# heliaxdev/ark-plonk

Measured on AMD Instinct MI355X. Metric: proofs/sec at 2^20 constraints (BLS12-381, KZG10); MSM G1-adds/s, higher is better.
Workload: dtype u32 limbs (256/384-bit Montgomery integers)

## Files before the change

### ark_plonk_amd/csrc/fieldu.cuh

```cuda
#pragma once
#include "field_common.cuh"

template <class P>
struct Fu {
    static constexpr int NL = P::NL;
    static constexpr int SAT = P::SAT_WORDS;
    static constexpr uint32_t M = (1u << 29) - 1u;
    uint32_t v[NL];

    ZK_HD static Fu zero() {
        Fu r;
#pragma unroll
        for (int i = 0; i < NL; ++i) r.v[i] = 0;
        return r;
    }
    ZK_HD static Fu one() {
        Fu r;
#pragma unroll
        for (int i = 0; i < NL; ++i) r.v[i] = P::ONE(i);
        return r;
    }
    ZK_HD bool limbs_zero() const {
        uint32_t o = 0;
#pragma unroll
        for (int i = 0; i < NL; ++i) o |= v[i];
        return o == 0;
    }

    ZK_HD static void normalize(Fu& t) {
#pragma unroll
        for (int i = 0; i < NL - 1; ++i) {
            uint32_t c = (uint32_t)((int32_t)t.v[i] >> 29);
            t.v[i] &= M;
            t.v[i + 1] += c;
        }
    }

    ZK_HD static Fu add(const Fu& a, const Fu& b) {
        Fu t;
#pragma unroll
        for (int i = 0; i < NL; ++i) t.v[i] = a.v[i] + b.v[i];
        normalize(t);
        return t;
    }
    ZK_HD static Fu dbl(const Fu& a) {
        Fu t;
#pragma unroll
        for (int i = 0; i < NL; ++i) t.v[i] = a.v[i] << 1;
        normalize(t);
        return t;
    }
    ZK_HD static Fu add3(const Fu& a, const Fu& b, const Fu& c) {
        Fu t;
#pragma unroll
        for (int i = 0; i < NL; ++i) t.v[i] = a.v[i] + b.v[i] + c.v[i];
        normalize(t);
        return t;
    }
    ZK_HD static Fu sub2(const Fu& a, const Fu& b) {
        Fu t;
#pragma unroll
        for (int i = 0; i < NL; ++i) t.v[i] = a.v[i] - b.v[i] + P::Z2(i);
        normalize(t);
        return t;
    }
    ZK_HD static Fu sub8(const Fu& a, const Fu& b) {
        Fu t;
#pragma unroll
        for (int i = 0; i < NL; ++i) t.v[i] = a.v[i] - b.v[i] + P::Z8(i);
        normalize(t);
        return t;
    }
    ZK_HD static Fu sub16(const Fu& a, const Fu& b) {
        Fu t;
#pragma unroll
        for (int i = 0; i < NL; ++i) t.v[i] = a.v[i] - b.v[i] + P::Z16(i);
        normalize(t);
        return t;
    }
    ZK_HD static Fu neg16(const Fu& a) {
        Fu t;
#pragma unroll
        for (int i = 0; i < NL; ++i) t.v[i] = P::Z16(i) - a.v[i];
        normalize(t);
        return t;
    }
    ZK_HD static Fu neg_canonical(const Fu& a) {
        Fu t;
#pragma unroll
        for (int i = 0; i < NL; ++i) t.v[i] = P::ZP(i) - a.v[i];
        normalize(t);
        return t;
    }

    ZK_HD static void sweep(Fu& t) {
#pragma unroll
        for (int i = 0; i < NL - 1; ++i) {
            const uint32_t c = t.v[i] >> 29;
            t.v[i] &= M;
            t.v[i + 1] += c;
        }
    }
    ZK_HD static Fu add_raw(const Fu& a, const Fu& b) {
        Fu t;
#pragma unroll
        for (int i = 0; i < NL; ++i) t.v[i] = a.v[i] + b.v[i];
        return t;
    }
    ZK_HD static Fu sub_raw3(const Fu& a, const Fu& b) {
        Fu t;
#pragma unroll
        for (int i = 0; i < NL; ++i) t.v[i] = a.v[i] + P::ZB3(i) - b.v[i];
        return t;
    }
    ZK_HD static Fu sub_raw8(const Fu& a, const Fu& b) {
        Fu t;
#pragma unroll
        for (int i = 0; i < NL; ++i) t.v[i] = a.v[i] + P::ZB8(i) - b.v[i];
        return t;
    }
    ZK_HD static Fu sub_raw16(const Fu& a, const Fu& b) {
        Fu t;
#pragma unroll
        for (int i = 0; i < NL; ++i) t.v[i] = a.v[i] + P::ZB16(i) - b.v[i];
        return t;
    }

    ZK_HD static Fu mul(const Fu& a, const Fu& b) {
        uint32_t m[NL];
        Fu r;
        uint64_t carry = 0;
#pragma unroll
        for (int k = 0; k < NL; ++k) {
            uint64_t a0 = 0, a1 = 0, am = 0;
#pragma unroll
            for (int i = 0; i <= k; ++i) {
                if (i & 1) a1 += (uint64_t)a.v[i] * b.v[k - i];
                else a0 += (uint64_t)a.v[i] * b.v[k - i];
            }
#pragma unroll
            for (int i = 0; i < k; ++i) am += (uint64_t)m[i] * P::MOD(k - i);
            uint64_t t = a0 + a1 + am + carry;
            m[k] = ((uint32_t)t * P::PINV) & M;
            t += (uint64_t)m[k] * P::MOD(0);
            carry = t >> 29;
        }
#pragma unroll
        for (int k = NL; k < 2 * NL - 1; ++k) {
            uint64_t a0 = 0, a1 = 0, am = 0;
#pragma unroll
            for (int i = k - NL + 1; i < NL; ++i) {
                if (i & 1) a1 += (uint64_t)a.v[i] * b.v[k - i];
                else a0 += (uint64_t)a.v[i] * b.v[k - i];
                am += (uint64_t)m[i] * P::MOD(k - i);
            }
            uint64_t t = a0 + a1 + am + carry;
            r.v[k - NL] = (uint32_t)t & M;
            carry = t >> 29;
        }
        r.v[NL - 1] = (uint32_t)carry;
        return r;
    }
    ZK_HD static uint64_t fence64(uint64_t t) {
#if defined(__HIP_DEVICE_COMPILE__)
        asm("" : "+v"(t));
#endif
        return t;
    }
    ZK_HD static Fu mul_fenced(const Fu& a, const Fu& b) {
        uint32_t m[NL];
        Fu r;
        uint64_t carry = 0;
#pragma unroll
        for (int k = 0; k < NL; ++k) {
            uint64_t t = fence64(carry + (uint64_t)a.v[0] * b.v[k]);
#pragma unroll
            for (int i = 1; i <= k; ++i) t += (uint64_t)a.v[i] * b.v[k - i];
#pragma unroll
            for (int i = 0; i < k; ++i) t += (uint64_t)m[i] * P::MOD(k - i);
            m[k] = ((uint32_t)t * P::PINV) & M;
            t += (uint64_t)m[k] * P::MOD(0);
            carry = t >> 29;
        }
#pragma unroll
        for (int k = NL; k < 2 * NL - 1; ++k) {
            uint64_t t = fence64(carry + (uint64_t)a.v[k - NL + 1] * b.v[NL - 1]);
#pragma unroll
            for (int i = k - NL + 2; i < NL; ++i) t += (uint64_t)a.v[i] * b.v[k - i];
#pragma unroll
            for (int i = k - NL + 1; i < NL; ++i) t += (uint64_t)m[i] * P::MOD(k - i);
            r.v[k - NL] = (uint32_t)t & M;
            carry = t >> 29;
        }
        r.v[NL - 1] = (uint32_t)carry;
        return r;
    }
    ZK_HD static Fu sqr(const Fu& a) {
        uint32_t m[NL], a2[NL];
        Fu r;
#pragma unroll
        for (int i = 0; i < NL; ++i) a2[i] = a.v[i] << 1;
        uint64_t carry = 0;
#pragma unroll
        for (int k = 0; k < NL; ++k) {
            uint64_t aa = 0, am = 0;
#pragma unroll
            for (int i = 0; 2 * i < k; ++i) aa += (uint64_t)a2[i] * a.v[k - i];
            if ((k & 1) == 0) aa += (uint64_t)a.v[k / 2] * a.v[k / 2];
#pragma unroll
            for (int i = 0; i < k; ++i) am += (uint64_t)m[i] * P::MOD(k - i);
            uint64_t t = aa + am + carry;
            m[k] = ((uint32_t)t * P::PINV) & M;
            t += (uint64_t)m[k] * P::MOD(0);
            carry = t >> 29;
        }
#pragma unroll
        for (int k = NL; k < 2 * NL - 1; ++k) {
            uint64_t aa = 0, am = 0;
#pragma unroll
            for (int i = k - NL + 1; 2 * i < k; ++i) aa += (uint64_t)a2[i] * a.v[k - i];
            if ((k & 1) == 0) aa += (uint64_t)a.v[k / 2] * a.v[k / 2];
#pragma unroll
            for (int i = k - NL + 1; i < NL; ++i) am += (uint64_t)m[i] * P::MOD(k - i);
            uint64_t t = aa + am + carry;
            r.v[k - NL] = (uint32_t)t & M;
            carry = t >> 29;
        }
        r.v[NL - 1] = (uint32_t)carry;
        return r;
    }

    ZK_HD bool is_zero_mod_reduced() const {
        if (v[0] != 0 && v[0] != P::MOD(0)) return false;
        uint32_t dz = 0, dp = 0;
#pragma unroll
        for (int i = 0; i < NL; ++i) {
            dz |= v[i];
            dp |= v[i] ^ P::MOD(i);
        }
        return dz == 0 || dp == 0;
    }
    ZK_HD bool is_zero_mod() const { return mul(*this, one()).is_zero_mod_reduced(); }

    ZK_HD static Fu canonical_lt2p(const Fu& a) {
        Fu d;
#pragma unroll
        for (int i = 0; i < NL; ++i) d.v[i] = a.v[i] - P::MOD(i);
        normalize(d);
        const bool neg = ((int32_t)d.v[NL - 1]) < 0;
        Fu r;
#pragma unroll
        for (int i = 0; i < NL; ++i) r.v[i] = neg ? a.v[i] : d.v[i];
        return r;
    }

    ZK_HD static Fu from_sat(const uint32_t* w) {
        Fu t = split_words(w);
        Fu c;
#pragma unroll
        for (int i = 0; i < NL; ++i) c.v[i] = P::C_IN(i);
        return mul(t, c);
    }
    ZK_HD void to_sat(uint32_t* w) const {
        Fu c;
#pragma unroll
        for (int i = 0; i < NL; ++i) c.v[i] = P::C_OUT(i);
        Fu t = canonical_lt2p(mul(*this, c));
        t.pack_words(w);
    }
    ZK_HD static Fu split_words(const uint32_t* w) {
        Fu t;
#pragma unroll
        for (int i = 0; i < NL; ++i) {
            const int bit = 29 * i;
            const int wi = bit >> 5, off = bit & 31;
            uint64_t lo = wi < SAT ? w[wi] : 0u;
            uint64_t hi = (wi + 1) < SAT ? w[wi + 1] : 0u;
            t.v[i] = (uint32_t)(((hi << 32) | lo) >> off) & M;
        }
        return t;
    }
    ZK_HD void pack_words(uint32_t* w) const { zk_pack_words<29>(*this, w); }

    ZK_HD static Fu pow_words(const Fu& a, const uint32_t* e, int n) { return zk_pow_words(a, e, n); }
    ZK_HD static Fu inverse(const Fu& a) {
        Fu pm;
#pragma unroll
        for (int i = 0; i < NL; ++i) pm.v[i] = P::MOD(i);
        uint32_t e[SAT];
        pm.pack_words(e);
        zk_words_minus_two(e);
        return zk_pow_words(a, e, SAT);
    }
};
```

### ark_plonk_amd/csrc/ntt.hip

```cpp
#include "ctx.h"
#include "domain.cuh"

#include "ntt_pass.cuh"

namespace {

template <class Fr>
struct PowBits {
    Fr p[32];
};
template <class Fr>
__global__ void gen_pow_table(void* out, uint64_t n, PowBits<Fr> pb, Fr mul, int mode, uint32_t log_m, uint32_t log_mprev, Fr to_rp) {
    uint64_t i = (uint64_t)blockIdx.x * blockDim.x + threadIdx.x;
    if (i >= n) return;
    uint64_t e = i;
    if (mode == 1) {
        uint64_t col = i & ((1ull << log_m) - 1);
        uint64_t k = i >> log_m;
        e = (col * k) & ((1ull << log_mprev) - 1);
    }
    Fr r = mul;
    for (int b = 0; b < 32; ++b) {
        if ((e >> b) & 1ull) r = Fr::mul(r, pb.p[b]);
    }
    st_fr<Fr>(out, i, Fr::mul(r, to_rp));
}

template <class FU>
__global__ void split_table(const void* packed, void* out, uint64_t n) {
    const uint64_t i = (uint64_t)blockIdx.x * blockDim.x + threadIdx.x;
    if (i >= n) return;
    const FU x = ld_u<FU>(packed, i);
    uint32_t w[4 * TW_INNER_U4];
#pragma unroll
    for (int k = 0; k < 4 * TW_INNER_U4; ++k) w[k] = k < FU::NL ? x.v[k] : 0u;
    uint4* q = reinterpret_cast<uint4*>(out) + TW_INNER_U4 * i;
#pragma unroll
    for (int k = 0; k < TW_INNER_U4; ++k) q[k] = make_uint4(w[4 * k], w[4 * k + 1], w[4 * k + 2], w[4 * k + 3]);
}

template <class Fr>
__global__ void ntt_tiny(const void* in, void* out, uint64_t in_len, uint32_t log_n, Fr w , Fr pre_g ,
                         Fr post_g , Fr scale ) {
    if (threadIdx.x != 0 || blockIdx.x != 0) return;
    const uint32_t n = 1u << log_n;
    Fr x[4], y[4];
    Fr gp = Fr::one();
    for (uint32_t i = 0; i < n; ++i) {
        x[i] = i < in_len ? Fr::mul(ld_fr<Fr>(in, i), gp) : Fr::zero();
        gp = Fr::mul(gp, pre_g);
    }
    Fr wi = Fr::one(), pg = scale;
    for (uint32_t i = 0; i < n; ++i) {
        Fr acc = Fr::zero(), wij = Fr::one();
        for (uint32_t j = 0; j < n; ++j) {
            acc = Fr::add(acc, Fr::mul(x[j], wij));
            wij = Fr::mul(wij, wi);
        }
        y[i] = Fr::mul(acc, pg);
        pg = Fr::mul(pg, post_g);
        wi = Fr::mul(wi, w);
    }
    for (uint32_t i = 0; i < n; ++i) st_fr<Fr>(out, i, y[i]);
}

template <class Fr>
__global__ void fr_convert_kernel(const void* in, void* out, uint64_t n, int to_mont) {
    uint64_t i = (uint64_t)blockIdx.x * blockDim.x + threadIdx.x;
    if (i >= n) return;
    Fr x = ld_fr<Fr>(in, i);
    st_fr<Fr>(out, i, to_mont ? Fr::to_mont(x) : Fr::from_mont(x));
}
template <class Fr>
__global__ void fr_mul_kernel(const void* a, const void* b, void* out, uint64_t n) {
    uint64_t i = (uint64_t)blockIdx.x * blockDim.x + threadIdx.x;
    if (i >= n) return;
    st_fr<Fr>(out, i, Fr::mul(ld_fr<Fr>(a, i), ld_fr<Fr>(b, i)));
}

template <class Fr>
PowBits<Fr> make_powbits(Fr base) {
    PowBits<Fr> pb;
    Fr cur = base;
    for (int b = 0; b < 32; ++b) {
        pb.p[b] = cur;
        cur = Fr::sqr(cur);
    }
    return pb;
}

template <class C>
int launch_pow_table(zk_ctx* c, void* out, uint64_t n, typename C::Fr base, typename C::Fr mul, int mode, uint32_t log_m,
                     uint32_t log_mprev) {
    typedef typename C::Fr Fr;
    if (n == 0) return ZK_OK;
    PowBits<Fr> pb = make_powbits(base);
    const Fr to_rp = to_rprime(Fr::one());
    const int T = 256;
    uint64_t blocks = (n + T - 1) / T;
    hipLaunchKernelGGL(gen_pow_table<Fr>, dim3((unsigned)blocks), dim3(T), 0, c->stream, out, n, pb, mul, mode, log_m, log_mprev, to_rp);
    ZK_HIP_TRY(hipGetLastError());
    return ZK_OK;
}

bool decompose(uint32_t log_n, int forced, int& n_pass, int s[4]) {
    s[0] = s[1] = s[2] = s[3] = 0;
    if (forced == 0 && log_n <= 9) {
        n_pass = 1;
        s[0] = (int)log_n;
        return true;
    }
    n_pass = forced ? forced : (int)((log_n + 8) / 9);
    if (n_pass > 4) return true;
    int base = (int)log_n / n_pass, extra = (int)log_n % n_pass;
    for (int i = 0; i < n_pass; ++i) s[i] = base + (i < extra ? 1 : 0);
    return forced == 0 || (s[n_pass - 1] >= 3 && s[0] <= 9);
}
int forced_passes(const zk_ctx* c, uint32_t log_n) { return log_n < 3 ? 0 : c->tune.ntt_passes; }

template <class C>
int get_inner_tw(zk_ctx* c, int s, bool inverse, void** out) {
    typedef typename C::Fr Fr;
    uint64_t key = ((uint64_t)C::ID << 40) | ((uint64_t)(inverse ? 1 : 0) << 32) | (uint64_t)s;
    auto it = c->inner_tw.find(key);
    if (it != c->inner_tw.end()) {
        *out = it->second;
        return ZK_OK;
    }
    uint64_t cnt = s >= 1 ? (1ull << (s - 1)) : 1;
    void* packed = nullptr;
    void* p = nullptr;
    ZK_HIP_TRY(hipMalloc(&packed, cnt * sizeof(Fr)));
    if (hipMalloc(&p, cnt * TW_INNER_U4 * 16) != hipSuccess) {
        (void)hipFree(packed);
        return ZK_ERR_OOM;
    }
    Fr w = domain_root<C>((uint32_t)s);
    if (inverse) w = Fr::inverse(w);
    int rc = launch_pow_table<C>(c, packed, cnt, w, Fr::one(), 0, 0, 0);
    if (!rc) {
        const int T = 256;
        hipLaunchKernelGGL(split_table<typename C::FrU>, dim3((unsigned)((cnt + T - 1) / T)), dim3(T), 0, c->stream, packed, p, cnt);
        if (hipGetLastError() != hipSuccess || hipStreamSynchronize(c->stream) != hipSuccess) rc = ZK_ERR_HIP;
    }
    (void)hipFree(packed);
    if (rc) {
        (void)hipFree(p);
        return rc;
    }
    c->inner_tw[key] = p;
    *out = p;
    return ZK_OK;
}

template <class C>
int get_plan(zk_ctx* c, uint32_t log_n, bool inverse, NttPlan** out) {
    typedef typename C::Fr Fr;
    const int forced = forced_passes(c, log_n);
    uint64_t key = ((uint64_t)C::ID << 40) | ((uint64_t)forced << 36) | ((uint64_t)(inverse ? 1 : 0) << 32) | log_n;
    auto it = c->plans.find(key);
    if (it != c->plans.end()) {
        *out = it->second;
        return ZK_OK;
    }
    int n_pass, s[4];
    if (!decompose(log_n, forced, n_pass, s)) return ZK_ERR_UNSUPPORTED;
    NttPlan* pl = new NttPlan();
    pl->curve = C::ID;
    pl->log_n = log_n;
    pl->inverse = inverse;
    pl->n_pass = n_pass;
    for (int i = 0; i < 4; ++i) pl->s[i] = s[i];
    uint32_t log_mprev = log_n;
    for (int p = 0; p < pl->n_pass; ++p) {
        if (log_n >= 3) {
            int rc = get_inner_tw<C>(c, pl->s[p], inverse, &pl->tw_inner[p]);
            if (rc) { delete pl; return rc; }
        }
        if (p + 1 < pl->n_pass) {
            uint32_t log_m = log_mprev - (uint32_t)pl->s[p];
            uint64_t cnt = 1ull << log_mprev;
            hipError_t e = hipMalloc(&pl->tw_pass[p], cnt * sizeof(Fr));
            if (e != hipSuccess) { delete pl; return ZK_ERR_OOM; }
            Fr w = domain_root<C>(log_mprev);
            if (inverse) w = Fr::inverse(w);
            int rc = launch_pow_table<C>(c, pl->tw_pass[p], cnt, w, Fr::one(), 1, log_m, log_mprev);
            if (rc) { delete pl; return rc; }
            log_mprev = log_m;
        }
    }
    c->plans[key] = pl;
    *out = pl;
    return ZK_OK;
}

template <class C>
int ensure_coset(zk_ctx* c, bool inv, uint64_t len, void** out) {
    typedef typename C::Fr Fr;
    DevBuf& buf = inv ? c->coset_inv_pow[C::ID] : c->coset_pow[C::ID];
    size_t& have = inv ? c->coset_inv_len[C::ID] : c->coset_len[C::ID];
    if (have < len) {
        ZK_HIP_TRY(hipStreamSynchronize(c->stream));
        uint64_t want = 1;
        while (want < len) want <<= 1;
        int rc = buf.ensure(want * sizeof(Fr));
        if (rc) return rc;
        Fr g = coset_gen<C>();
        if (inv) g = Fr::inverse(g);
        rc = launch_pow_table<C>(c, buf.p, want, g, Fr::one(), 0, 0, 0);
        if (rc) return rc;
        have = want;
    }
    *out = buf.p;
    return ZK_OK;
}

typedef int (*NttPassLauncher)(int final_pass, const NttPassArgs* a, hipStream_t st);
extern "C" NttPassLauncher zk_ntt_pass_launcher(int curve, int s);

template <class C>
int dispatch_pass(zk_ctx* c, int s, bool final_pass, const NttPassArgs& a) {
    if (s < 3 || s > 9) return ZK_ERR_UNSUPPORTED;
    NttPassLauncher fn = zk_ntt_pass_launcher(C::ID, s);
    if (!fn) return ZK_ERR_UNSUPPORTED;
    hipError_t e = (hipError_t)fn(final_pass ? 1 : 0, &a, c->stream);
    ZK_HIP_TRY(e);
    return ZK_OK;
}

template <class C>
int ntt_run(zk_ctx* c, int kind, uint32_t log_n, uint32_t n_polys, const void* const* d_ins, const size_t* in_lens, void* const* d_outs) {
    typedef typename C::Fr Fr;
    if (!domain_log_ok<C>(log_n)) return ZK_ERR_DOMAIN_TOO_LARGE;
    if (n_polys == 0 || n_polys > 16) return ZK_ERR_BAD_ARG;
    const uint64_t N = 1ull << log_n;
    size_t in_len = 0;
    bool all_quarter = true;
    for (uint32_t i = 0; i < n_polys; ++i) {
        if (in_lens[i] > N) return ZK_ERR_BAD_ARG;
        if (in_lens[i] > in_len) in_len = in_lens[i];
        if ((uint64_t)in_lens[i] * 4 > N) all_quarter = false;
    }
    const void* d_in = d_ins[0];
    void* d_out = d_outs[0];
    const bool inverse = (kind == ZK_NTT_IFFT || kind == ZK_NTT_COSET_IFFT);
    int rc;
    Fr n_inv = Fr::inverse(Fr::from_u64(N));
    if (log_n < 3) {
        Fr w = domain_root<C>(log_n);
        if (inverse) w = Fr::inverse(w);
        Fr g = coset_gen<C>();
        Fr pre_g = kind == ZK_NTT_COSET_FFT ? g : Fr::one();
        Fr post_g = kind == ZK_NTT_COSET_IFFT ? Fr::inverse(g) : Fr::one();
        ProfScope ps(c, "ntt_pass");
        for (uint32_t i = 0; i < n_polys; ++i)
            hipLaunchKernelGGL(ntt_tiny<Fr>, dim3(1), dim3(64), 0, c->stream, d_ins[i], d_outs[i], (uint64_t)in_lens[i], log_n, w, pre_g, post_g,
                               inverse ? n_inv : Fr::one());
        ZK_HIP_TRY(hipGetLastError());
        return ZK_OK;
    }
    {
        int np, sp[4];
        if (!decompose(log_n, forced_passes(c, log_n), np, sp)) return ZK_ERR_UNSUPPORTED;
    }
    void* pre = nullptr;
    void* post = nullptr;
    if (kind == ZK_NTT_COSET_FFT && in_len > 0) {
        rc = ensure_coset<C>(c, false, in_len, &pre);
        if (rc) return rc;
    }
    if (kind == ZK_NTT_COSET_IFFT) {
        rc = ensure_coset<C>(c, true, N, &post);
        if (rc) return rc;
    }
    NttPlan* pl = nullptr;
    rc = get_plan<C>(c, log_n, inverse, &pl);
    if (rc) return rc;
    if (pl->n_pass > 4) return ZK_ERR_UNSUPPORTED;
    void* work = nullptr;
    if (pl->n_pass > 1) {
        rc = c->ntt_work.ensure((size_t)n_polys * N * sizeof(Fr));
        if (rc) return rc;
        work = c->ntt_work.p;
    }
    uint32_t log_mprev = log_n;
    NttPassArgs a;
    ProfScope ps(c, "ntt_pass");
    for (int p = 0; p < pl->n_pass; ++p) {
        const int s = pl->s[p];
        const bool last = (p + 1 == pl->n_pass);
        memset(&a, 0, sizeof a);
        a.log_n = log_n;
        a.in = (p == 0) ? d_in : work;
        a.out = last ? d_out : work;
        a.in_len = (p == 0) ? in_lens[0] : N;
        if (n_polys > 1) {
            a.n_batch = n_polys;
            for (uint32_t i = 0; i < n_polys; ++i) {
                void* wk = (char*)work + (size_t)i * N * sizeof(Fr);
                a.ins[i] = (p == 0) ? d_ins[i] : wk;
                a.outs[i] = last ? d_outs[i] : wk;
                a.in_lens[i] = (p == 0) ? in_lens[i] : N;
            }
        }
        a.tw_inner = pl->tw_inner[p];
        a.pre_mul = (p == 0) ? pre : nullptr;
        const uint32_t LC = 9u - (uint32_t)s;
        if (!last) {
            uint32_t log_m = log_mprev - (uint32_t)s;
            uint32_t logc = LC < log_m ? LC : log_m;
            a.logc = logc;
            a.log_m = log_m;
            a.log_mprev = log_mprev;
            a.tw_pass = pl->tw_pass[p];
            a.n_tiles = (uint32_t)(N >> ((uint32_t)s + logc));
            a.quarter = (p == 0 && s >= 3 && all_quarter) ? 1u : 0u;
            log_mprev = log_m;
        } else {
            uint32_t s1 = (pl->n_pass > 1) ? (uint32_t)pl->s[0] : 0;
            uint32_t logc = LC < s1 ? LC : s1;
            a.logc = logc;
            a.s1 = s1;
            a.s2 = pl->n_pass == 4 ? (uint32_t)pl->s[1] : 0u;
            a.post_mul = post;
            const Fr sc = to_rprime(inverse ? n_inv : Fr::one());
            for (int i = 0; i < 8; ++i) a.scale[i] = sc.v[i];
            a.n_tiles = (uint32_t)(N >> ((uint32_t)s + logc));
        }
        rc = dispatch_pass<C>(c, s, last, a);
        if (rc) return rc;
        if (c->profiling) c->prof["ntt_passes"].launches += 1;
    }
    return ZK_OK;
}

}

int ntt_run_dev(zk_ctx* c, int curve, int kind, uint32_t log_n, const void* d_in, size_t in_len, void* d_out) {
    return ntt_run_batch_dev(c, curve, kind, log_n, 1, &d_in, &in_len, &d_out);
}

int ntt_run_batch_dev(zk_ctx* c, int curve, int kind, uint32_t log_n, uint32_t n_polys, const void* const* d_ins, const size_t* in_lens,
                      void* const* d_outs) {
    if (kind < 0 || kind > 3) return ZK_ERR_BAD_ARG;
    for (uint32_t base = 0; base < n_polys; base += 16) {
        const uint32_t cnt = n_polys - base < 16 ? n_polys - base : 16;
        const int rc = zk_on_curve(curve, ZK_ERR_BAD_ARG, [&](auto cv) {
            return ntt_run<decltype(cv)>(c, kind, log_n, cnt, d_ins + base, in_lens + base, d_outs + base);
        });
        if (rc) return rc;
    }
    return ZK_OK;
}

int ntt_prepare(zk_ctx* c, int curve, uint32_t log_n) {
    NttPlan* pl;
    if (log_n < 3) return ZK_OK;
    for (int inv = 0; inv < 2; ++inv) {
        const int rc = zk_on_curve(curve, ZK_ERR_BAD_ARG, [&](auto cv) {
            typedef decltype(cv) Cv;
            if (!domain_log_ok<Cv>(log_n)) return ZK_ERR_DOMAIN_TOO_LARGE;
            return get_plan<Cv>(c, log_n, inv != 0, &pl);
        });
        if (rc) return rc;
    }
    return ZK_OK;
}

void ntt_ctx_free(zk_ctx* c) {
    for (auto& kv : c->plans) delete kv.second;
    c->plans.clear();
    for (auto& kv : c->inner_tw) (void)hipFree(kv.second);
    c->inner_tw.clear();
    c->ntt_work.release();
    for (int i = 0; i < 2; ++i) {
        c->coset_pow[i].release();
        c->coset_inv_pow[i].release();
    }
}

static int fr_convert_on(int curve, int to_mont, const void* d_in, size_t n, void* d_out, hipStream_t st) {
    if (n == 0) return ZK_OK;
    const int T = 256;
    unsigned blocks = (unsigned)((n + T - 1) / T);
    const int rc = zk_on_curve(curve, ZK_ERR_BAD_ARG, [&](auto cv) {
        hipLaunchKernelGGL(fr_convert_kernel<typename decltype(cv)::Fr>, dim3(blocks), dim3(T), 0, st, d_in, d_out, (uint64_t)n, to_mont);
        return ZK_OK;
    });
    if (rc) return rc;
    ZK_HIP_TRY(hipGetLastError());
    return ZK_OK;
}
int fr_convert_dev(zk_ctx* c, int curve, int to_mont, const void* d_in, size_t n, void* d_out) {
    return fr_convert_on(curve, to_mont, d_in, n, d_out, c->stream);
}
int fr_convert_stream(zk_ctx* c, int curve, const void* d_in, size_t n, void* d_out, hipStream_t st) {
    (void)c;
    return fr_convert_on(curve, 0, d_in, n, d_out, st);
}

int fr_mul_dev(zk_ctx* c, int curve, const void* a, const void* b, size_t n, void* out) {
    if (n == 0) return ZK_OK;
    const int T = 256;
    unsigned blocks = (unsigned)((n + T - 1) / T);
    const int rc = zk_on_curve(curve, ZK_ERR_BAD_ARG, [&](auto cv) {
        hipLaunchKernelGGL(fr_mul_kernel<typename decltype(cv)::Fr>, dim3(blocks), dim3(T), 0, c->stream, a, b, out, (uint64_t)n);
        return ZK_OK;
    });
    if (rc) return rc;
    ZK_HIP_TRY(hipGetLastError());
    return ZK_OK;
}
```

### ark_plonk_amd/csrc/ntt_pass.cuh

```cuda
#pragma once
#include <hip/hip_runtime.h>
#include "curve_params.h"
#include "field.cuh"
#include "fieldu.cuh"

typedef __attribute__((address_space(3))) volatile uint32_t lds_u32;

struct NttPassArgs {
    const void* in;
    void* out;
    const void* tw_inner;
    const void* tw_pass;
    const void* pre_mul;
    const void* post_mul;
    uint32_t scale[8];
    uint64_t in_len;
    uint32_t log_n;
    uint32_t logc;
    uint32_t log_m;
    uint32_t log_mprev;
    uint32_t s1;
    uint32_t s2;
    uint32_t n_tiles;
    uint32_t quarter;
    uint32_t n_batch;
    const void* ins[16];
    void* outs[16];
    uint64_t in_lens[16];
};

__host__ __device__ inline uint32_t bitrev32(uint32_t x, int bits) {
#if defined(__HIP_DEVICE_COMPILE__)
    return bits ? __brev(x) >> (32 - bits) : 0u;
#else
    uint32_t r = 0;
    for (int i = 0; i < bits; ++i) { r = (r << 1) | (x & 1); x >>= 1; }
    return r;
#endif
}

template <class F>
ZK_D F ld_u(const void* base, uint64_t idx) {
    const uint4* q = reinterpret_cast<const uint4*>(base) + 2 * idx;
    uint4 a = q[0], b = q[1];
    uint32_t w[8] = {a.x, a.y, a.z, a.w, b.x, b.y, b.z, b.w};
    return F::split_words(w);
}
template <class F>
ZK_D void st_u(void* base, uint64_t idx, const F& x) {
    uint32_t w[8];
    F::canonical_lt2p(x).pack_words(w);
    uint4* q = reinterpret_cast<uint4*>(base) + 2 * idx;
    q[0] = make_uint4(w[0], w[1], w[2], w[3]);
    q[1] = make_uint4(w[4], w[5], w[6], w[7]);
}

template <class F>
ZK_D void st_u_raw(void* base, uint64_t idx, const F& x) {
    uint32_t w[8];
    x.pack_words(w);
    uint4* q = reinterpret_cast<uint4*>(base) + 2 * idx;
    q[0] = make_uint4(w[0], w[1], w[2], w[3]);
    q[1] = make_uint4(w[4], w[5], w[6], w[7]);
}

constexpr int TW_INNER_U4 = 3;
template <class F>
ZK_D F ld_limbs(const void* base, uint64_t idx) {
    static_assert(F::NL <= 4 * TW_INNER_U4, "inner twiddle entry too small");
    const uint4* q = reinterpret_cast<const uint4*>(base) + TW_INNER_U4 * idx;
    F r;
#pragma unroll
    for (int i = 0; i < TW_INNER_U4; ++i) {
        if (4 * i >= F::NL) break;
        const uint4 a = q[i];
        if (4 * i + 0 < F::NL) r.v[4 * i + 0] = a.x;
        if (4 * i + 1 < F::NL) r.v[4 * i + 1] = a.y;
        if (4 * i + 2 < F::NL) r.v[4 * i + 2] = a.z;
        if (4 * i + 3 < F::NL) r.v[4 * i + 3] = a.w;
    }
    return r;
}

constexpr int ntt_units_before(int t) {
    int b = 1;
    for (int s = 0; s < t; ++s) {
        if (b > 6) b = 1;
        b += 2;
    }
    return b;
}
constexpr bool ntt_sweep_at(int t) { return ntt_units_before(t) > 6; }
static_assert(ntt_units_before(1) == 3 && ntt_units_before(2) == 5 && ntt_units_before(3) == 7 && ntt_units_before(4) == 3, "two units per stage");
static_assert(!ntt_sweep_at(0) && !ntt_sweep_at(2) && ntt_sweep_at(3) && !ntt_sweep_at(5) && ntt_sweep_at(6) && ntt_sweep_at(9), "a sweep every third stage");

template <int B0>
ZK_D uint32_t window_pos(uint32_t v, uint32_t e) {
    return ((v >> B0) << (B0 + 3)) | (e << B0) | (v & ((1u << B0) - 1u));
}

template <class F>
ZK_D void wave_exchange(F (&x)[8], lds_u32* sc, const uint32_t (&widx)[8], const uint32_t (&ridx)[8]) {
#pragma unroll
    for (int l = 0; l < F::NL; ++l) {
#pragma unroll
        for (int e = 0; e < 8; ++e) sc[widx[e]] = x[e].v[l];
        __builtin_amdgcn_wave_barrier();
#pragma unroll
        for (int e = 0; e < 8; ++e) x[e].v[l] = sc[ridx[e]];
        __builtin_amdgcn_wave_barrier();
    }
}

template <class F, int S, int B0, int LB_LO, int LB_HI>
ZK_D void dit_window(F (&x)[8], uint32_t v, const void* tw, bool quarter) {
    const uint32_t vlow = v & ((1u << B0) - 1u);
#pragma unroll
    for (int lb = LB_LO; lb < LB_HI; ++lb) {
        const int t = B0 + lb;
        if (ntt_sweep_at(t)) {
#pragma unroll
            for (int e = 0; e < 8; ++e) F::sweep(x[e]);
        }
#pragma unroll
        for (int e = 0; e < 8; ++e) {
            if (e & (1 << lb)) continue;
            const int eo = e | (1 << lb);
            if constexpr (B0 == 0 && LB_LO == 0) {
                if (lb < 2 && quarter) {
                    x[eo] = x[e];
                    continue;
                }
                if (lb == 0) {
                    const F b = x[eo];
                    x[eo] = F::sub_raw3(x[e], b);
                    x[e] = F::add_raw(x[e], b);
                    continue;
                }
                if ((e & ((1 << lb) - 1)) == 0) {
                    F b = x[eo];
                    F::sweep(b);
                    x[eo] = lb == 1 ? F::sub_raw8(x[e], b) : F::sub_raw16(x[e], b);
                    x[e] = F::add_raw(x[e], b);
                    continue;
                }
            }
            const uint32_t plow = ((uint32_t)(e & ((1 << lb) - 1)) << B0) | vlow;
            const uint32_t j = plow << (S - 1 - t);
            F w = ld_limbs<F>(tw, j);
            F m = F::mul_fenced(x[eo], w);
            x[eo] = F::sub_raw3(x[e], m);
            x[e] = F::add_raw(x[e], m);
        }
    }
}

template <class F, int S, int B0>
ZK_D void dit_all(F (&x)[8], uint32_t v, uint32_t c, uint32_t LC, const void* tw, lds_u32* sc, bool quarter = false) {
    constexpr int REM = S - B0;
    if constexpr (REM >= 3) {
        dit_window<F, S, B0, 0, 3>(x, v, tw, quarter);
        if constexpr (REM > 3) {
            constexpr int NB0 = (REM - 3 >= 3) ? B0 + 3 : S - 3;
            uint32_t wi[8], ri[8];
#pragma unroll
            for (int e = 0; e < 8; ++e) {
                wi[e] = (window_pos<B0>(v, e) << LC) | c;
                ri[e] = (window_pos<NB0>(v, e) << LC) | c;
            }
            wave_exchange<F>(x, sc, wi, ri);
            if constexpr (REM - 3 >= 3) {
                dit_all<F, S, B0 + 3>(x, v, c, LC, tw, sc);
            } else {
                dit_window<F, S, S - 3, 3 - (REM - 3), 3>(x, v, tw, false);
            }
        }
    }
}

template <class F, int S>
__global__ void __launch_bounds__(256) ntt_pass_mid(NttPassArgs a) {
    constexpr uint32_t LC = 9 - S;
    __shared__ uint32_t scratch[4][512];
    const uint32_t lane = threadIdx.x & 63, wv = threadIdx.x >> 6;
    const uint32_t tile = blockIdx.x * (blockDim.x >> 6) + wv;
    if (tile >= a.n_tiles) return;
    const void* in = a.in;
    void* out = a.out;
    uint64_t in_len = a.in_len;
    if (a.n_batch) {
        in = a.ins[blockIdx.y];
        out = a.outs[blockIdx.y];
        in_len = a.in_lens[blockIdx.y];
    }
    lds_u32* sc = (lds_u32*)scratch[wv];
    const uint32_t c = lane & ((1u << LC) - 1u);
    const uint32_t v = lane >> LC;
    const bool active = c < (1u << a.logc);
    const uint32_t lcg = a.log_m - a.logc;
    const uint64_t blk = (uint64_t)tile >> lcg;
    const uint64_t cg = (uint64_t)tile & ((1ull << lcg) - 1);
    const uint64_t col = (cg << a.logc) + c;
    const uint64_t base = (blk << a.log_mprev) + col;

    F x[8];
#pragma unroll
    for (int e = 0; e < 8; ++e) {
        const uint64_t row = bitrev32((v << 3) | e, S);
        const uint64_t idx = base + (row << a.log_m);
        if (active && idx < in_len) {
            x[e] = ld_u<F>(in, idx);
            if (a.pre_mul) x[e] = F::mul_fenced(x[e], ld_u<F>(a.pre_mul, idx));
        } else {
            x[e] = F::zero();
        }
    }
    dit_all<F, S, 0>(x, v, c, LC, a.tw_inner, sc, a.quarter != 0);
    if (!active) return;
#pragma unroll
    for (int e = 0; e < 8; ++e) {
        const uint64_t k = S >= 3 ? (((uint64_t)e << (S - 3)) | v) : e;
        F w = ld_u<F>(a.tw_pass, (k << a.log_m) + col);
        if (ntt_units_before(S) > 6) F::sweep(x[e]);
        st_u_raw<F>(out, base + (k << a.log_m), F::mul_fenced(x[e], w));
    }
}

template <class F, int S>
__global__ void __launch_bounds__(256) ntt_pass_final(NttPassArgs a) {
    constexpr uint32_t L = 1u << S;
    constexpr uint32_t LC = 9 - S;
    __shared__ uint32_t scratch[4][512];
    const uint32_t lane = threadIdx.x & 63, wv = threadIdx.x >> 6;
    const uint32_t tile = blockIdx.x * (blockDim.x >> 6) + wv;
    if (tile >= a.n_tiles) return;
    const void* in = a.in;
    void* out = a.out;
    uint64_t in_len = a.in_len;
    if (a.n_batch) {
        in = a.ins[blockIdx.y];
        out = a.outs[blockIdx.y];
        in_len = a.in_lens[blockIdx.y];
    }
    lds_u32* sc = (lds_u32*)scratch[wv];
    const uint32_t log_nb = a.log_n - S;
    const uint32_t log_rest = log_nb - a.s1;
    const uint32_t lg = a.s1 - a.logc;
    const uint64_t rho = (uint64_t)tile >> lg;
    const uint64_t g = (uint64_t)tile & ((1ull << lg) - 1);

    F x[8];
    uint32_t wi[8], ri[8];
    const uint32_t c = lane & ((1u << LC) - 1u);
    const uint32_t v = lane >> LC;
#pragma unroll
    for (int e = 0; e < 8; ++e) {
        const uint32_t q = (uint32_t)e * 64u + lane;
        const uint32_t cb = q >> S, row = q & (L - 1);
        const uint64_t b = ((((uint64_t)g << a.logc) + cb) << log_rest) | rho;
        const uint64_t idx = (b << S) + row;
        if (cb < (1u << a.logc) && idx < in_len) {
            x[e] = ld_u<F>(in, idx);
            if (a.pre_mul) x[e] = F::mul_fenced(x[e], ld_u<F>(a.pre_mul, idx));
        } else {
            x[e] = F::zero();
        }
        wi[e] = (bitrev32(row, S) << LC) | cb;
        ri[e] = (((v << 3) | (uint32_t)e) << LC) | c;
    }
    wave_exchange<F>(x, sc, wi, ri);
    dit_all<F, S, 0>(x, v, c, LC, a.tw_inner, sc);
    if (c >= (1u << a.logc)) return;
    const uint64_t k1o = ((uint64_t)g << a.logc) + c;
    uint64_t rho_rev = rho;
    if (a.s2) {
        const uint32_t s3 = log_rest - a.s2;
        rho_rev = (rho >> s3) | ((rho & ((1ull << s3) - 1ull)) << a.s2);
    }
    const uint64_t obase = k1o + (rho_rev << a.s1);
    F sc_mul = F::split_words(a.scale);
#pragma unroll
    for (int e = 0; e < 8; ++e) {
        const uint64_t k = S >= 3 ? (((uint64_t)e << (S - 3)) | v) : e;
        const uint64_t oidx = obase + (k << log_nb);
        if (ntt_units_before(S) > 6) F::sweep(x[e]);
        F y = F::mul_fenced(x[e], sc_mul);
        if (a.post_mul) y = F::mul_fenced(y, ld_u<F>(a.post_mul, oidx));
        st_u<F>(out, oidx, y);
    }
}
```

Measured before the change: 12.96.

## Fold inverse-NTT 1/n scale into pass twiddles and drop final Montgomery multiply

```diff
diff --git a/ark_plonk_amd/csrc/fieldu.cuh b/ark_plonk_amd/csrc/fieldu.cuh
--- a/ark_plonk_amd/csrc/fieldu.cuh
+++ b/ark_plonk_amd/csrc/fieldu.cuh
@@ -254,6 +254,45 @@
         return r;
     }
 
+    ZK_HD static void canonical_words_lt48p(const Fu& a, uint32_t* w) {
+        constexpr uint32_t PT = P::MOD(NL - 1);
+        static_assert(PT >= (1u << 21) && 48ull * (PT + 1) <= (1ull << 29), "quotient estimate: 2^53 / (pt + 1) in a word, 48 p below 2^(29 NL)");
+        constexpr uint32_t G = (uint32_t)((1ull << 53) / ((uint64_t)PT + 1));
+        Fu pm;
+#pragma unroll
+        for (int i = 0; i < NL; ++i) pm.v[i] = P::MOD(i);
+        uint32_t pw[SAT], x[SAT], y[SAT], z[SAT];
+        pm.pack_words(pw);
+        a.pack_words(x);
+        const uint32_t q = (uint32_t)(((uint64_t)a.v[NL - 1] * G) >> 53);
+        uint32_t hi = 0, bw = 0;
+#pragma unroll
+        for (int j = 0; j < SAT; ++j) {
+            const uint64_t c = (uint64_t)q * pw[j] + hi;
+            const uint32_t lo = (uint32_t)c;
+            hi = (uint32_t)(c >> 32);
+            const uint32_t d = x[j] - lo;
+            const uint32_t b1 = x[j] < lo;
+            y[j] = d - bw;
+            bw = b1 | (uint32_t)(d < bw);
+        }
+        bw = 0;
+#pragma unroll
+        for (int j = 0; j < SAT; ++j) {
+            const uint32_t d = y[j] - pw[j];
+            const uint32_t b1 = y[j] < pw[j];
+            z[j] = d - bw;
+            bw = b1 | (uint32_t)(d < bw);
+        }
+#pragma unroll
+        for (int j = 0; j < SAT; ++j) w[j] = bw ? y[j] : z[j];
+    }
+    ZK_HD static Fu canonical_lt48p(const Fu& a) {
+        uint32_t w[SAT];
+        canonical_words_lt48p(a, w);
+        return split_words(w);
+    }
+
     ZK_HD static Fu from_sat(const uint32_t* w) {
         Fu t = split_words(w);
         Fu c;
diff --git a/ark_plonk_amd/csrc/ntt.hip b/ark_plonk_amd/csrc/ntt.hip
--- a/ark_plonk_amd/csrc/ntt.hip
+++ b/ark_plonk_amd/csrc/ntt.hip
@@ -184,7 +184,9 @@
             if (e != hipSuccess) { delete pl; return ZK_ERR_OOM; }
             Fr w = domain_root<C>(log_mprev);
             if (inverse) w = Fr::inverse(w);
-            int rc = launch_pow_table<C>(c, pl->tw_pass[p], cnt, w, Fr::one(), 1, log_m, log_mprev);
+            const bool fold = inverse && p + 2 == pl->n_pass;
+            const Fr mul = fold ? Fr::inverse(Fr::from_u64(1ull << log_n)) : Fr::one();
+            int rc = launch_pow_table<C>(c, pl->tw_pass[p], cnt, w, mul, 1, log_m, log_mprev);
             if (rc) { delete pl; return rc; }
             log_mprev = log_m;
         }
@@ -323,8 +325,11 @@
             a.s1 = s1;
             a.s2 = pl->n_pass == 4 ? (uint32_t)pl->s[1] : 0u;
             a.post_mul = post;
-            const Fr sc = to_rprime(inverse ? n_inv : Fr::one());
-            for (int i = 0; i < 8; ++i) a.scale[i] = sc.v[i];
+            a.unscaled = pl->n_pass > 1 ? 1u : 0u;
+            if (!a.unscaled) {
+                const Fr sc = to_rprime(inverse ? n_inv : Fr::one());
+                for (int i = 0; i < 8; ++i) a.scale[i] = sc.v[i];
+            }
             a.n_tiles = (uint32_t)(N >> ((uint32_t)s + logc));
         }
         rc = dispatch_pass<C>(c, s, last, a);
diff --git a/ark_plonk_amd/csrc/ntt_pass.cuh b/ark_plonk_amd/csrc/ntt_pass.cuh
--- a/ark_plonk_amd/csrc/ntt_pass.cuh
+++ b/ark_plonk_amd/csrc/ntt_pass.cuh
@@ -23,6 +23,7 @@
     uint32_t s2;
     uint32_t n_tiles;
     uint32_t quarter;
+    uint32_t unscaled;
     uint32_t n_batch;
     const void* ins[16];
     void* outs[16];
@@ -50,6 +51,15 @@
 ZK_D void st_u(void* base, uint64_t idx, const F& x) {
     uint32_t w[8];
     F::canonical_lt2p(x).pack_words(w);
+    uint4* q = reinterpret_cast<uint4*>(base) + 2 * idx;
+    q[0] = make_uint4(w[0], w[1], w[2], w[3]);
+    q[1] = make_uint4(w[4], w[5], w[6], w[7]);
+}
+
+template <class F>
+ZK_D void st_u_lt48(void* base, uint64_t idx, const F& x) {
+    uint32_t w[8];
+    F::canonical_words_lt48p(x, w);
     uint4* q = reinterpret_cast<uint4*>(base) + 2 * idx;
     q[0] = make_uint4(w[0], w[1], w[2], w[3]);
     q[1] = make_uint4(w[4], w[5], w[6], w[7]);
@@ -278,13 +288,23 @@
         rho_rev = (rho >> s3) | ((rho & ((1ull << s3) - 1ull)) << a.s2);
     }
     const uint64_t obase = k1o + (rho_rev << a.s1);
+    if (a.unscaled && !a.post_mul) {
+#pragma unroll
+        for (int e = 0; e < 8; ++e) {
+            const uint64_t k = S >= 3 ? (((uint64_t)e << (S - 3)) | v) : e;
+            F::sweep(x[e]);
+            st_u_lt48<F>(out, obase + (k << log_nb), x[e]);
+        }
+        return;
+    }
     F sc_mul = F::split_words(a.scale);
 #pragma unroll
     for (int e = 0; e < 8; ++e) {
         const uint64_t k = S >= 3 ? (((uint64_t)e << (S - 3)) | v) : e;
         const uint64_t oidx = obase + (k << log_nb);
         if (ntt_units_before(S) > 6) F::sweep(x[e]);
-        F y = F::mul_fenced(x[e], sc_mul);
+        F y = x[e];
+        if (!a.unscaled) y = F::mul_fenced(y, sc_mul);
         if (a.post_mul) y = F::mul_fenced(y, ld_u<F>(a.post_mul, oidx));
         st_u<F>(out, oidx, y);
     }
```

Result: no change. 13.03, median of 6 (+0.5%).
